# 20171130/Equivariant-NN-Zoo

Measured on AMD Instinct MI355X. Metric: molecules/s forward+backward, QM9 config_energy batch, higher is better.
Workload: dtype f32

## Files before the change

equivariant-nn-zoo_amd/csrc/e3k_graph.hip:

```cpp
#include "e3k_common.h"

namespace e3k {

__global__ __launch_bounds__(256) void csr_count_kernel(const int64_t* __restrict__ edge_index, int64_t E, int32_t N,
                                                        int32_t* __restrict__ src, int32_t* __restrict__ dst,
                                                        int32_t* __restrict__ dst_ptr, int32_t* __restrict__ src_ptr,
                                                        int32_t* __restrict__ bad) {
  const int64_t e = (int64_t)blockIdx.x * 256 + threadIdx.x;
  if (e >= E) return;
  int64_t s = edge_index[e], d = edge_index[E + e];
  if (s < 0 || s >= N || d < 0 || d >= N) {
    *bad = 1;
    s = d = 0;
  }
  src[e] = (int32_t)s;
  dst[e] = (int32_t)d;
  atomicAdd(src_ptr + s + 1, 1);
  atomicAdd(dst_ptr + d + 1, 1);
}

__global__ __launch_bounds__(1024) void csr_scan_kernel(int32_t* __restrict__ dst_ptr, int32_t* __restrict__ src_ptr,
                                                        int32_t* __restrict__ dst_cur, int32_t* __restrict__ src_cur, int32_t N) {
  int32_t* ptr = blockIdx.x == 0 ? dst_ptr : src_ptr;
  int32_t* cur = blockIdx.x == 0 ? dst_cur : src_cur;
// ... 129 lines not shown
      bounds[2 * k] = acc;
      bounds[2 * k + 1] = count[k];
      acc += count[k];
    }
  }
  __syncthreads();
  for (int base = 0; base < R; base += 1024) {
    const int i = base + t;
    int k = -1;
    if (i < R) {
      const int64_t kk = key[i];
      k = (kk >= 0 && kk < K) ? (int)kk : -1;
    }
    int rank = 0;
    for (int q = 0; q < K; ++q) {
      const unsigned long long b = __ballot(k == q);
      if (k == q) rank = __popcll(b & ((1ull << lane) - 1ull));
      if (lane == 0) hist[w][q] = __popcll(b);
    }
    __syncthreads();
    int before[GR_EPT];
#pragma unroll
    for (int j = 0; j < GR_EPT; ++j) {
      const int e = t + 1024 * j, tw = e / K, tq = e - tw * K;
      before[j] = 0;
      if (e < 16 * K)
        for (int v = 0; v < tw; ++v) before[j] += hist[v][tq];
    }
    __syncthreads();
    int total_q[GR_EPT];
#pragma unroll
    for (int j = 0; j < GR_EPT; ++j) {
      const int e = t + 1024 * j, tw = e / K, tq = e - tw * K;
      total_q[j] = 0;
      if (e < 16 * K) {
        if (tw == 15) total_q[j] = before[j] + hist[15][tq];
        hist[tw][tq] = before[j];
      }
    }
    __syncthreads();
    if (k >= 0) perm[start[k] + running[k] + hist[w][k] + rank] = i;
    __syncthreads();
#pragma unroll
    for (int j = 0; j < GR_EPT; ++j) {
      const int e = t + 1024 * j, tw = e / K, tq = e - tw * K;
      if (e < 16 * K && tw == 15) running[tq] += total_q[j];
    }
    __syncthreads();
  }
  if (t < K) reps[t] = count[t] > 0 ? perm[start[t]] : 0;
}
}

namespace e3k {
__global__ __launch_bounds__(256) void edge_records_kernel(const int32_t* __restrict__ perm, const int32_t* __restrict__ nbr,
                                                           const int32_t* __restrict__ bin, const float* __restrict__ coef,
                                                           const float* __restrict__ sh, int d_sh, int64_t E, int32_t* __restrict__ rec) {
  const int64_t q = (int64_t)blockIdx.x * 256 + threadIdx.x;
  if (q >= E * 16) return;
  const int64_t t = q >> 4;
  const int f = (int)(q & 15);
  const int e = perm[t];
  int32_t v = 0;
  if (f == 0) v = nbr[e];
  else if (f == 1) v = bin ? bin[e] : 0;
  else if (f < 6) v = coef ? __float_as_int(coef[4 * (int64_t)e + (f - 2)]) : 0;
  else if (f < 15) v = (f - 6) < d_sh ? __float_as_int(sh[(int64_t)e * d_sh + (f - 6)]) : 0;
  else v = e;
  rec[q] = v;
}
}

extern "C" int e3k_edge_records(const int32_t* perm, const int32_t* nbr, const int32_t* bin, const float* coef, const float* sh,
                                int32_t d_sh, int64_t E, int32_t* rec, void* stream) {
  if (E < 0 || d_sh <= 0 || d_sh > 9 || (bin != nullptr) != (coef != nullptr)) return E3K_ERR_INVALID;
  if (E >= 0x7fffffffLL) return E3K_ERR_UNSUPPORTED;
  if (E == 0) return E3K_OK;
  if (!perm || !nbr || !sh || !rec || (reinterpret_cast<uintptr_t>(rec) & 63)) return E3K_ERR_INVALID;
  hipLaunchKernelGGL(e3k::edge_records_kernel, dim3((unsigned)((E * 16 + 255) / 256)), dim3(256), 0, (hipStream_t)stream, perm, nbr, bin,
                     coef, sh, d_sh, E, rec);
  E3K_CHECK_LAUNCH();
  return E3K_OK;
}

extern "C" int e3k_group_rows(const int64_t* key, int64_t R, int32_t K, int32_t* perm, int32_t* bounds, int64_t* reps,
                              int32_t* bad_flag, void* stream) {
  if (R < 0 || K <= 0) return E3K_ERR_INVALID;
  if (K > e3k::GR_MAXK || R >= 0x7fffffffLL) return E3K_ERR_UNSUPPORTED;
  if (!bounds || !reps || !bad_flag || (R > 0 && (!key || !perm))) return E3K_ERR_INVALID;
  hipStream_t st = (hipStream_t)stream;
  hipLaunchKernelGGL(e3k::group_rows_kernel, dim3(1), dim3(1024), 0, st, key, (int32_t)R, K, perm, bounds, reps, bad_flag);
  E3K_CHECK_LAUNCH();
  return E3K_OK;
}
```

equivariant-nn-zoo_amd/csrc/e3k_rtable.hip:

```cpp
#include "e3k_common.h"
#include "e3k_rtable_bwd.h"

namespace e3k {


constexpr int RT_CHUNK = 1024;
__global__ __launch_bounds__(256) void rtable_bins_rank_kernel(const float* __restrict__ r, const int64_t* __restrict__ key, int64_t E,
                                                               float h_inv, int32_t K, int32_t KT, int32_t* __restrict__ bin,
                                                               float* __restrict__ coef, int32_t* __restrict__ lrank,
                                                               int32_t* __restrict__ chunk_hist, int32_t* __restrict__ bad) {
  extern __shared__ int32_t hist_all[];
  const int lane = threadIdx.x & 63, wv = threadIdx.x >> 6;
  int32_t* hist = hist_all + wv * (KT + 1);
  const int64_t chunk = blockIdx.x;
  for (int b = threadIdx.x; b < 4 * (KT + 1); b += 256) hist_all[b] = 0;
  __syncthreads();
  constexpr int PER_WAVE = RT_CHUNK / 4 / 64;
  const int64_t base = chunk * RT_CHUNK + (int64_t)wv * (RT_CHUNK / 4);
  int my_bin[PER_WAVE], my_rank[PER_WAVE];
#pragma unroll
  for (int it = 0; it < PER_WAVE; ++it) {
    const int64_t e = base + it * 64 + lane;
    const bool live = e < E;
    int i = 1;
    if (live) {
      const float raw = r[e] * h_inv;
      float x = raw < 0.f ? 0.f : (raw > (float)K ? (float)K : raw);
      i = (int)x;
      i = i < 1 ? 1 : (i > K - 2 ? K - 2 : i);
      const float t = x - (float)i;
      const float tm1 = t - 1.f, tm2 = t - 2.f, tp1 = t + 1.f;
      float4 c;
      c.x = -t * tm1 * tm2 * (1.f / 6.f);
      c.y = tp1 * tm1 * tm2 * 0.5f;
      c.z = -tp1 * t * tm2 * 0.5f;
      c.w = tp1 * t * tm1 * (1.f / 6.f);
      if (key) {
        const int64_t kk = key[e];
        const int nk = (KT + 1) / (K + 1);
        const bool in_range = kk >= 0 && kk < nk;
        i += in_range ? (int)kk * (K + 1) : 0;
        if (!in_range && bad) atomicOr(bad, 8);
      }
      bin[e] = i;
      *reinterpret_cast<float4*>(coef + 4 * e) = c;
    }
    unsigned long long todo = __ballot(live);
    int rank = 0;
    while (todo) {
      const int leader = __ffsll((long long)todo) - 1;
      const int b = __shfl(i, leader, 64);
      const unsigned long long same = __ballot(live && i == b) & todo;
      const int seen = hist[b];
      if (live && i == b) rank = seen + __popcll(same & ((1ull << lane) - 1ull));
      if (lane == leader) hist[b] = seen + __popcll(same);
      todo &= ~same;
    }
    my_bin[it] = live ? i : -1;
    my_rank[it] = rank;
  }
  __syncthreads();
#pragma unroll
  for (int it = 0; it < PER_WAVE; ++it) {
    if (my_bin[it] < 0) continue;
    int before = 0;
    for (int w = 0; w < wv; ++w) before += hist_all[w * (KT + 1) + my_bin[it]];
    lrank[base + it * 64 + lane] = my_rank[it] + before;
  }
  for (int b = threadIdx.x; b <= KT; b += 256)
    chunk_hist[chunk * (KT + 1) + b] = hist_all[b] + hist_all[(KT + 1) + b] + hist_all[2 * (KT + 1) + b] + hist_all[3 * (KT + 1) + b];
}

__global__ __launch_bounds__(1024) void rtable_bins_scan_kernel(int32_t* __restrict__ chunk_hist, int32_t n_chunks, int32_t K,
                                                                int32_t* __restrict__ ptr, int32_t* __restrict__ seg) {
  __shared__ int32_t wave_tot[2][16];
  __shared__ int32_t carry[2];
  const int t = threadIdx.x, lane = t & 63, w = t >> 6;
  if (t < 2) carry[t] = 0;
  __syncthreads();
  for (int base = 0; base <= K; base += 1024) {
    const int b = base + t;
    int32_t cnt = 0;
    if (b <= K) {
      for (int c = 0; c < n_chunks; ++c) {
        const int32_t v = chunk_hist[(int64_t)c * (K + 1) + b];
        chunk_hist[(int64_t)c * (K + 1) + b] = cnt;
        cnt += v;
      }
    }
    const int32_t sg = (cnt + RT_SEG - 1) / RT_SEG;
    int32_t x = cnt, y = sg;
#pragma unroll
    for (int off = 1; off < 64; off <<= 1) {
      const int32_t xx = __shfl_up(x, off, 64), yy = __shfl_up(y, off, 64);
      if (lane >= off) x += xx, y += yy;
    }
    if (lane == 63) wave_tot[0][w] = x, wave_tot[1][w] = y;
    __syncthreads();
    int32_t bx = carry[0], by = carry[1];
    for (int k = 0; k < w; ++k) bx += wave_tot[0][k], by += wave_tot[1][k];
    if (b <= K) {
      ptr[b] = bx + x - cnt;
      seg[b] = by + y - sg;
      if (b == K) ptr[K + 1] = bx + x, seg[K + 1] = by + y;
    }
    __syncthreads();
    if (t == 1023) carry[0] = bx + x, carry[1] = by + y;
    __syncthreads();
  }
}

__global__ __launch_bounds__(256) void rtable_bins_place_kernel(const int32_t* __restrict__ bin, const int32_t* __restrict__ lrank,
                                                                const int32_t* __restrict__ chunk_off, const int32_t* __restrict__ ptr,
                                                                int64_t E, int32_t K, int32_t* __restrict__ perm) {
  const int64_t e = (int64_t)blockIdx.x * 256 + threadIdx.x;
  if (e >= E) return;
  const int b = bin[e];
  perm[ptr[b] + chunk_off[(e / RT_CHUNK) * (K + 1) + b] + lrank[e]] = (int32_t)e;
}

__global__ __launch_bounds__(256) void rtable_interp_fwd_kernel(const float* __restrict__ T, const int32_t* __restrict__ perm,
                                                                const int32_t* __restrict__ bin, const float* __restrict__ coef,
                                                                int64_t E, int32_t W, float* __restrict__ w,
                                                                const float* __restrict__ T2, float* __restrict__ w2) {
  const int64_t p = (int64_t)blockIdx.x * 4 + (threadIdx.x >> 6);
  if (p >= E) return;
  const int lane = threadIdx.x & 63;
  const int e = uniform(perm[p]);
  const int i = uniform(bin[e]);
  const float* __restrict__ cp = coef + 4 * (int64_t)e;
  const float c0 = __uint_as_float(uniform((int)__float_as_uint(cp[0]))), c1 = __uint_as_float(uniform((int)__float_as_uint(cp[1])));
  const float c2 = __uint_as_float(uniform((int)__float_as_uint(cp[2]))), c3 = __uint_as_float(uniform((int)__float_as_uint(cp[3])));
  const float4* __restrict__ a = reinterpret_cast<const float4*>(T + (int64_t)(i - 1) * W);
  const float4* __restrict__ b = reinterpret_cast<const float4*>(T + (int64_t)i * W);
  const float4* __restrict__ c = reinterpret_cast<const float4*>(T + (int64_t)(i + 1) * W);
  const float4* __restrict__ d = reinterpret_cast<const float4*>(T + (int64_t)(i + 2) * W);
  float4* __restrict__ o = reinterpret_cast<float4*>(w + (int64_t)e * W);
  for (int q = lane; q < (W >> 2); q += 64) {
    const float4 va = a[q], vb = b[q], vc = c[q], vd = d[q];
    float4 v;
// ... 254 lines not shown
}

extern "C" int e3k_rtable_pack(const float* T, int32_t K, int32_t W, void* P, void* stream) {
  if (K < 4 || W <= 0) return E3K_ERR_INVALID;
  if (!T || !P) return E3K_ERR_INVALID;
  const int64_t q = (int64_t)(K + 1) * W;
  hipLaunchKernelGGL(e3k::rtable_pack_kernel, dim3((unsigned)((q + 255) / 256)), dim3(256), 0, (hipStream_t)stream, T, K, W,
                     static_cast<uint32_t*>(P));
  E3K_CHECK_LAUNCH();
  return E3K_OK;
}

extern "C" int e3k_rtable_pack_multi(const float* const* T, int32_t K, const int32_t* W, void* const* P, int32_t n, void* stream) {
  if (K < 4 || n < 0 || n > 16) return E3K_ERR_INVALID;
  if (n == 0) return E3K_OK;
  if (!T || !W || !P) return E3K_ERR_INVALID;
  e3k::PackMulti a{};
  int32_t wmax = 0;
  for (int i = 0; i < n; ++i) {
    if (!T[i] || !P[i] || W[i] <= 0) return E3K_ERR_INVALID;
    a.T[i] = T[i];
    a.P[i] = static_cast<uint32_t*>(P[i]);
    a.W[i] = W[i];
    wmax = W[i] > wmax ? W[i] : wmax;
  }
  const int64_t q = (int64_t)(K + 1) * wmax;
  hipLaunchKernelGGL(e3k::rtable_pack_multi_kernel, dim3((unsigned)((q + 255) / 256), (unsigned)n), dim3(256), 0, (hipStream_t)stream, a, K);
  E3K_CHECK_LAUNCH();
  return E3K_OK;
}

extern "C" int e3k_rtable_interp_packed(const void* P, const int32_t* bin_perm, const int32_t* bin, const float* coef, int64_t E,
                                        int32_t K, int32_t W, float* w, void* stream) {
  if (E < 0 || K < 4 || W <= 0) return E3K_ERR_INVALID;
  if (E >= 0x7fffffffLL) return E3K_ERR_UNSUPPORTED;
  if (E == 0) return E3K_OK;
  if (!P || !bin_perm || !bin || !coef || !w) return E3K_ERR_INVALID;
  hipLaunchKernelGGL(e3k::rtable_interp_packed_kernel, dim3((unsigned)((E + 3) / 4)), dim3(256), 0, (hipStream_t)stream,
                     static_cast<const uint32_t*>(P), bin_perm, bin, coef, E, W, w);
  E3K_CHECK_LAUNCH();
  return E3K_OK;
}

extern "C" int64_t e3k_rtable_bins_workspace_ints(int64_t E, int32_t K) {
  const int64_t n_chunks = (E + e3k::RT_CHUNK - 1) / e3k::RT_CHUNK;
  return E + n_chunks * ((int64_t)K + 1);
}

static int rtable_bins_impl(const float* r, const int64_t* key, int32_t n_keys, int64_t E, float h_inv, int32_t K, int32_t* bin,
                            float* coef, int32_t* bin_ptr, int32_t* bin_seg, int32_t* bin_perm, int32_t* workspace, int32_t* bad_flag,
                            void* stream) {
  if (E < 0 || K < 4 || !(h_inv > 0.f) || n_keys < 1) return E3K_ERR_INVALID;
  const int64_t KT64 = (int64_t)n_keys * (K + 1) - 1;
  if (KT64 > 4000 || E >= 0x7fffffffLL) return E3K_ERR_UNSUPPORTED;
  const int32_t KT = (int32_t)KT64;
  if (!bin_ptr || !bin_seg) return E3K_ERR_INVALID;
  if (E > 0 && (!r || !bin || !coef || !bin_perm || !workspace)) return E3K_ERR_INVALID;
  hipStream_t st = (hipStream_t)stream;
  const int64_t n_chunks = (E + e3k::RT_CHUNK - 1) / e3k::RT_CHUNK;
  int32_t* lrank = workspace;
  int32_t* chunk_hist = workspace + E;
  if (E > 0)
    hipLaunchKernelGGL(e3k::rtable_bins_rank_kernel, dim3((unsigned)n_chunks), dim3(256), sizeof(int32_t) * 4 * (KT + 1), st, r, key, E,
                       h_inv, K, KT, bin, coef, lrank, chunk_hist, bad_flag);
  hipLaunchKernelGGL(e3k::rtable_bins_scan_kernel, dim3(1), dim3(1024), 0, st, chunk_hist, (int32_t)n_chunks, KT, bin_ptr, bin_seg);
  if (E > 0)
    hipLaunchKernelGGL(e3k::rtable_bins_place_kernel, dim3((unsigned)((E + 255) / 256)), dim3(256), 0, st, bin, lrank, chunk_hist,
                       bin_ptr, E, KT, bin_perm);
  E3K_CHECK_LAUNCH();
  return E3K_OK;
}

extern "C" int e3k_rtable_bins(const float* r, int64_t E, float h_inv, int32_t K, int32_t* bin, float* coef,
                               int32_t* bin_ptr, int32_t* bin_seg, int32_t* bin_perm, int32_t* workspace, void* stream) {
  return rtable_bins_impl(r, nullptr, 1, E, h_inv, K, bin, coef, bin_ptr, bin_seg, bin_perm, workspace, nullptr, stream);
}

extern "C" int e3k_rtable_bins_keyed(const float* r, const int64_t* key, int32_t n_keys, int64_t E, float h_inv, int32_t K,
                                     int32_t* bin, float* coef, int32_t* bin_ptr, int32_t* bin_seg, int32_t* bin_perm,
                                     int32_t* workspace, int32_t* bad_flag, void* stream) {
  if (E > 0 && !key) return E3K_ERR_INVALID;
  return rtable_bins_impl(r, key, n_keys, E, h_inv, K, bin, coef, bin_ptr, bin_seg, bin_perm, workspace, bad_flag, stream);
}

extern "C" int e3k_rtable_interp_fwd(const float* T, const int32_t* bin_perm, const int32_t* bin, const float* coef, int64_t E,
                                     int32_t K, int32_t W, float* w, void* stream) {
  if (E < 0 || K < 4 || W <= 0) return E3K_ERR_INVALID;
  if (W % 4 || E >= 0x7fffffffLL) return E3K_ERR_UNSUPPORTED;
  if (E == 0) return E3K_OK;
  if (!T || !bin_perm || !bin || !coef || !w) return E3K_ERR_INVALID;
  hipLaunchKernelGGL(e3k::rtable_interp_fwd_kernel, dim3((unsigned)((E + 3) / 4)), dim3(256), 0, (hipStream_t)stream, T, bin_perm,
                     bin, coef, E, W, w, (const float*)nullptr, (float*)nullptr);
  E3K_CHECK_LAUNCH();
  return E3K_OK;
}

extern "C" int e3k_rtable_interp_fwd2(const float* T, const float* T2, const int32_t* bin_perm, const int32_t* bin, const float* coef,
                                      int64_t E, int32_t K, int32_t W, float* w, float* w2, void* stream) {
  if (E < 0 || K < 4 || W <= 0) return E3K_ERR_INVALID;
  if (W % 4 || E >= 0x7fffffffLL) return E3K_ERR_UNSUPPORTED;
  if (E == 0) return E3K_OK;
  if (!T || !T2 || !bin_perm || !bin || !coef || !w || !w2) return E3K_ERR_INVALID;
  hipLaunchKernelGGL(e3k::rtable_interp_fwd_kernel, dim3((unsigned)((E + 3) / 4)), dim3(256), 0, (hipStream_t)stream, T, bin_perm,
                     bin, coef, E, W, w, T2, w2);
  E3K_CHECK_LAUNCH();
  return E3K_OK;
}
// ... 27 lines not shown
```

equivariant-nn-zoo_amd/e3_layers_amd/backend/radial_table.py:

```python
from __future__ import annotations

import os
import weakref
from typing import Optional

import torch

from .tuning import knob as _knob

from . import lib as L
from . import memo, ops

ENABLED = _knob("E3K_RADIAL_TABLE")
KNOTS = _knob("E3K_RADIAL_KNOTS")
KNOTS_SLOPE = _knob("E3K_RADIAL_KNOTS_SLOPE")
MIN_EDGES_PER_KNOT = _knob("E3K_RADIAL_MIN_EDGES_PER_KNOT")
KNOTS_MAX = _knob("E3K_RADIAL_KNOTS_MAX")
_KNOTS_AT_START = (int(KNOTS), int(KNOTS_SLOPE))
REFINEMENTS = 0
KEYED = _knob("E3K_RADIAL_TABLE_KEYED")


def layout(r_max: float, target: int):
    import math

    m = math.ceil(math.log2(max(int(target), 4) / float(r_max)) - 1e-9)
    h = 2.0 ** (-m)
    return max(int(math.ceil(float(r_max) / h - 1e-9)), 4), h


class KnotBins:

    __slots__ = ("bin", "coef", "ptr", "perm", "seg", "knots", "spacing", "blocks", "_buf", "_rec", "__weakref__")

    def __init__(self, bin, coef, ptr, perm, seg, knots: int, spacing: float, buf=None):
        self.bin, self.coef, self.ptr, self.perm, self.seg, self.knots, self.spacing = bin, coef, ptr, perm, seg, int(knots), float(spacing)
        self._buf = buf
        self._rec = {}
        self.blocks = 1

    def records(self, topo, sh: torch.Tensor, walk: str) -> torch.Tensor:
        perm, nbr = (topo.dst_perm, topo.src) if walk == "dst" else (topo.src_perm, topo.dst)
        key = (walk, sh.data_ptr(), sh._version, perm.data_ptr())
        hit = self._rec.get(key)
        if hit is None:
            sh = L.f32c(sh.detach())
            e = perm.numel()
            if sh.dim() != 2 or sh.shape[0] != e or sh.shape[1] > 9:
                raise ValueError(f"edge records take [E, <= 9] spherical harmonics, got {tuple(sh.shape)} for {e} edges")
            rec = torch.empty(max(e, 1), 16, dtype=torch.int32, device=sh.device)
            L.check(L.load().e3k_edge_records(L.ptr(perm), L.ptr(nbr), L.ptr(self.bin), L.ptr(self.coef), L.ptr(sh), sh.shape[1], e,
                                              L.ptr(rec), L.stream_ptr()), "e3k_edge_records")
            hit = self._rec[key] = (rec, sh)
        return hit[0]

    def tensors(self):
        return (self._buf, self.coef) if self._buf is not None else (self.bin, self.coef, self.ptr, self.perm, self.seg)

    def __iter__(self):
        return iter(self.tensors())


def build_bins(r: torch.Tensor, r_max: float, target: int, key: Optional[torch.Tensor] = None, n_keys: int = 1) -> KnotBins:
    knots, h = layout(r_max, target)
    r = L.f32c(r.detach().reshape(-1))
    L.require_cuda(r)
    e, dev = r.numel(), r.device
    lib = L.load()
    n_keys = int(n_keys) if key is not None else 1
    last = n_keys * (knots + 1) - 1
    sizes = [e, e, last + 2, last + 2, int(lib.e3k_rtable_bins_workspace_ints(e, last))]
    buf = torch.empty(sum(sizes), dtype=torch.int32, device=dev)
    bin32, perm, ptr, seg, work = torch.split(buf, sizes)
    coef = torch.empty(e, 4, dtype=torch.float32, device=dev)
    if key is None:
        L.check(lib.e3k_rtable_bins(L.ptr(r), e, 1.0 / h, knots, L.ptr(bin32), L.ptr(coef), L.ptr(ptr), L.ptr(seg), L.ptr(perm),
                                    L.ptr(work), L.stream_ptr()), "e3k_rtable_bins")
    else:
        key = key.detach().reshape(-1)
        if key.dtype != torch.int64 or not key.is_contiguous():
            key = key.long().contiguous()
        if key.numel() != e:
            raise ValueError(f"{key.numel()} keys for {e} radii")
        from . import graph as _graph

        capturing = torch.cuda.is_current_stream_capturing()
        flag = _graph._capture_flags.get(dev.index) if capturing else _graph.persistent_flag(dev)
        L.check(lib.e3k_rtable_bins_keyed(L.ptr(r), L.ptr(key), n_keys, e, 1.0 / h, knots, L.ptr(bin32), L.ptr(coef), L.ptr(ptr),
                                          L.ptr(seg), L.ptr(perm), L.ptr(work), L.ptr(flag), L.stream_ptr()), "e3k_rtable_bins_keyed")
        if flag is not None:
            _graph.report_persistent(dev)
    bins = KnotBins(bin32, coef, ptr, perm, seg, last, h, buf)
    bins.blocks = n_keys
    return bins


class RadialSource:

    __slots__ = ("module", "r", "version", "knots", "knots_slope", "_bins", "_knot_basis", "_stack", "__weakref__")

    def __init__(self, module, r: torch.Tensor, version: int = 0, prepared: Optional[dict] = None):
        self.module, self.r, self.version = weakref.ref(module), r, int(version)
        self.knots, self.knots_slope = int(KNOTS), int(KNOTS_SLOPE)
        self._bins = dict(prepared) if prepared else {}
        self._knot_basis = {}
        self._stack = {}

# ... 408 lines not shown
```

equivariant-nn-zoo_amd/e3_layers_amd/nn/message_passing.py:

```python
from __future__ import annotations

import math
import os
import weakref

from typing import Callable, Dict, Optional, Tuple

import torch

from ..backend.tuning import knob as _knob
from torch import Tensor

from ..backend import conv_block, conv_native, memo, ops, radial_table
from ..backend.graph import get_topology
from ..o3 import Irrep, Irreps
from ..utils.utils import _is_mapping, activations, build, tp_path_exists
from .core import (FullyConnectedNet, FullyConnectedTensorProduct, Gate, Linear, NormActivation, get_row_key, irreps_blocks,
                   row_groups)
from .pointwise import LayerNormalization, TensorProductExpansion
from .sequential import Module


FWD_FORK = _knob("E3K_FWD_FORK")
FORK_MIN_EDGES = _knob("E3K_FORK_MIN_EDGES")
# ... 377 lines not shown
        if nmp is not None and fork and nmp.conv._fork_pays(n_edges, table is not None):
            plan_n = nmp._block_plan()
            if plan_n is not None and (nmp.conv.sc is None) == (conv.sc is None):
                fc_n = list(nmp.conv.fc.children())
                same_path = (table is not None) == radial_table.applicable(data["edge_radial"], fc_n[-1].weight)
                if fc_n[0].weight.shape[0] == radial.shape[1] and same_path:
                    nxt = (plan_n, fc_n[-1].weight, [m.weight for m in fc_n[:-1]])
        y = conv_block.conv_block(x, attrs, radial, sh, plan, topo, groups, bool(getattr(x, "_e3k_cf", False)), out_cf, fork,
                                  conv.linear_1.weight, conv.tp.linear.weight, conv.sc.weight if conv.sc is not None else None,
                                  fc[-1].weight, [m.weight for m in fc[:-1]], table=table, nxt=nxt, m_pre=m_pre)
        return y

    def _forward_block_addend(self, data, x, sh, radial, out_cf: bool):
        plan = self._block_plan(addend=True) if BLOCK_ADDEND else None
        if plan is None:
            return None
        conv = self.conv
        x_cf = x if getattr(x, "_e3k_cf", False) else ops.relayout(x, conv._in_blocks, True)
        sc_out = conv.sc(x_cf, data["node_attrs"])
        topo = get_topology(data, x.shape[0])
        fc = list(conv.fc.children())
        table = None
        if radial_table.applicable(radial, fc[-1].weight):
            src = radial_table.source_of(radial)
            table = src.bins()
            radial = src.knot_basis()
        fork = bool(FWD_FORK and conv._fork_pays(data["edge_radial"].shape[0], table is not None)
                    and not torch.cuda.is_current_stream_capturing())
        if fork:
            main = ops.current_stream(x.device)
            side = ops.side_stream(x.device)
            with ops.on_stream(side, main):
                radial = _stream_alias(radial, side)
        return conv_block.conv_block(x_cf, None, radial, sh, plan, topo, None, True, out_cf, fork,
                                     conv.linear_1.weight, conv.tp.linear.weight, None,
                                     fc[-1].weight, [m.weight for m in fc[:-1]], table=table, m_pre=sc_out)

    def prepare_batch(self, network, data, avail) -> None:
        from ..backend.graph import GraphTopo

        if not conv_native.TP_TABLE:
            return
        inv = {loc: g for g, loc in self.input_key_mapping.items()}
        sh_key, rad_key = inv.get("edge_spherical"), inv.get("edge_radial")
        sh = data.get(sh_key) if sh_key in avail else None
        topo = GraphTopo.from_dict(data)
        if sh is None or topo is None or not sh.is_cuda or sh.dim() != 2 or sh.shape[1] > 9 or sh.shape[0] != topo.num_edges:
            return
        for _, layer in network.layers:
            if rad_key in getattr(layer, "output_key_mapping", {}).values() and hasattr(layer, "basis"):
                r_key = next((g for g, loc in layer.input_key_mapping.items() if loc == "input"), None)
                bins = radial_table.prepared_bins(data[r_key], layer.basis.r_max) if (r_key in avail and r_key in data) else None
                for b in (bins or {}).values():
                    b.records(topo, sh, "dst")
                    if torch.is_grad_enabled() or self.training:
                        b.records(topo, sh, "src")

    def forward(self, data: Dict[str, Tensor], attrs: Dict[str, Tuple[str, str]]):
        old_x = data["input_features"]
        blk = self._forward_block(data, bool(self._emit_cf))
        if blk is not None:
            if self._emit_cf:
                if self.normalize:
                    blk = self.norm({"input": blk}, attrs)[0]["output"]
                blk._e3k_cf = True
                return ({"output_features": blk},
                        {"output_features": (attrs["input_features"][0], self.irreps_out["output_features"])})
            output = blk
            if self.resnet:
                output = old_x + output
            if self.normalize:
                output = self.norm({"input": output}, attrs)[0]["output"]
            return ({"output_features": output},
                    {"output_features": (attrs["input_features"][0], self.irreps_out["output_features"])})
        if isinstance(self.conv, FactorizedConvolution) and self.conv.reduce:
            conv_cf = self.conv.forward_cf(data)
        else:
            if getattr(old_x, "_e3k_cf", False):
                raise RuntimeError("cf hand-over reached a convolution that cannot take it (container bug)")
            out, _ = self.conv(data, attrs)
            conv_cf = ops.relayout(out["output_features"], tuple(irreps_blocks(self.equivariant_nonlin.irreps_in)), True)
        if self._emit_cf:
            output = self.equivariant_nonlin(conv_cf, out_cf=True)
            if self.normalize:
                output = self.norm({"input": output}, attrs)[0]["output"]
            output._e3k_cf = True
            return ({"output_features": output},
                    {"output_features": (attrs["input_features"][0], self.irreps_out["output_features"])})
        output = self.equivariant_nonlin(conv_cf)
        if self.resnet:
            output = old_x + output
        if self.normalize:
            output = self.norm({"input": output}, attrs)[0]["output"]
        return ({"output_features": output},
                {"output_features": (attrs["input_features"][0], self.irreps_out["output_features"])})
```

equivariant-nn-zoo_amd/e3_layers_amd/run/graph_step.py:

```python
from __future__ import annotations

import os
from typing import Any, Callable

import numpy as np
import torch

from ..backend import memo


class CapturedStep:
    def __init__(self, fn: Callable[[], Any], warmup: int = 3, device=None, generators=()):
        if not torch.cuda.is_available():
            raise RuntimeError("CapturedStep needs a HIP device: there is no CPU fallback for graph replay")
        self.fn = fn
        self.generators = tuple(generators)
        self.dev = torch.device("cuda", torch.cuda.current_device()) if device is None else torch.device(device)
        self.recaptures = 0
        self._capture(max(1, warmup))

    def _eager(self, n: int):
        dev = self.dev
        side = torch.cuda.Stream(dev)
        side.wait_stream(torch.cuda.current_stream(dev))
# ... 85 lines not shown
        elif name == "_n_nodes":
            tensors[name] = torch.full_like(v, n_nodes)
        elif name == "_n_edges":
            tensors[name] = torch.full_like(v, n_edges)
        elif torch.is_tensor(v) and (like.attrs.get(name, ("",))[0] == "node"
                                     or (name not in like.attrs and v.dim() >= 1 and v.shape[0] == like[key].shape[0])):
            tensors[name] = v[:1].expand(n_nodes, *v.shape[1:]).clone()
        elif name == "edge_cell_shift":
            tensors[name] = v.new_zeros((n_edges,) + tuple(v.shape[1:]))
        elif torch.is_tensor(v) and like.attrs.get(name, ("",))[0] == "edge":
            tensors[name] = (v[:1].expand(n_edges, *v.shape[1:]).clone() if v.shape[0] else v.new_zeros((n_edges,) + tuple(v.shape[1:])))
        elif torch.is_tensor(v):
            tensors[name] = torch.zeros_like(v)
        else:
            tensors[name] = v
    return Data(attrs=dict(like.attrs), **tensors)


def pad_batch(batch, n_cap: int, e_cap: int, key: str = "pos"):
    from ..data.data import Batch
    from ..data.loader import samples_of

    dev = batch[key].device
    samples = samples_of(batch)
    n, e = int(batch[key].shape[0]), int(batch["edge_index"].shape[1])
    if n_cap < n + 2 or e_cap < e:
        raise ValueError(f"batch with {n} nodes / {e} edges does not fit the bucket ({n_cap}, {e_cap}; two ghost nodes are the minimum)")
    samples.append(ghost_sample(samples[0], n_cap - n, e_cap - e, key))
    out = Batch.from_data_list(samples, attrs=dict(samples[0].attrs))
    w = torch.full((len(samples), 1), 1.0 / (len(samples) - 1), dtype=torch.float32)
    w[-1] = 0.0
    out["_graph_weight"] = w
    out.attrs["_graph_weight"] = ("graph", "1x0e")
    wn = torch.zeros(n_cap, 1, dtype=torch.float32)
    wn[:n] = 1.0 / n
    out["_node_weight"] = wn
    out.attrs["_node_weight"] = ("node", "1x0e")
    return out.to(dev)


GHOST_DEGREE = 16


def ghost_node_capacity(n: int, ghost_edges: int, multiple: int = 32) -> int:
    return -(-(n + max(2, -(-ghost_edges // GHOST_DEGREE))) // multiple) * multiple


def bucket_capacity(sizes, node_multiple: int = 32, edge_multiple: int = 1024):
    e_cap = -(-max(e for _, e in sizes) // edge_multiple) * edge_multiple
    return max(ghost_node_capacity(n, e_cap - e, node_multiple) for n, e in sizes), e_cap


def copy_into(static, padded, keys, hint: str = "") -> None:
    by_dtype = {}
    for k in keys:
        dst, src = static[k], padded[k]
        if dst.shape != src.shape:
            raise ValueError(f"{k}: {tuple(src.shape)} does not fit the captured {tuple(dst.shape)} (another bucket?"
                             f"{' ' + hint if hint else ''})")
        if src.device == dst.device and src.dtype == dst.dtype and src.is_contiguous() and dst.is_contiguous():
            pair = by_dtype.setdefault(dst.dtype, ([], []))
            pair[0].append(dst)
            pair[1].append(src)
        else:
            dst.copy_(src, non_blocking=True)
    for dsts, srcs in by_dtype.values():
        torch._foreach_copy_(dsts, srcs)


class BucketedStep:

    def __init__(self, fn: Callable[[Any], Any], example, warmup: int = 3, generators=(), tail: Callable[[], Any] = None):
        self.tail = tail
        self.static = example.clone()
        self.keys = [k for k in self.static.keys() if torch.is_tensor(self.static[k])]

        def captured_fn():
            memo.forget(self.static)
            return fn(self.static.view())

        self.captured = CapturedStep(captured_fn, warmup=warmup, generators=generators)

    @property
    def recaptures(self) -> int:
        return self.captured.recaptures

    def __call__(self, padded):
        copy_into(self.static, padded, self.keys)
        out = self.captured()
        if self.tail is not None:
            self.tail()
        return out


def stream_beside(main, candidates: int = 6):
    dev = main.device
    busy = torch.empty(16 << 20, device=dev)
    tiny = torch.zeros(64, device=dev)
    pool = [torch.cuda.Stream(dev) for _ in range(candidates)]
    for st in pool:
        torch.cuda.synchronize(dev)
        with torch.cuda.stream(main):
            for _ in range(40):
                busy.mul_(1.0)
            main_done = torch.cuda.Event()
            main_done.record(main)
        with torch.cuda.stream(st):
            tiny.add_(1.0)
            mine = torch.cuda.Event()
            mine.record(st)
        mine.synchronize()
        beside = not main_done.query()
        torch.cuda.synchronize(dev)
        if beside:
            return st
    return pool[0]


class PipelinedBucketedStep:

# ... 206 lines not shown
```

include/e3k.h:

```cpp
#ifndef E3K_H
#define E3K_H

#include <stdint.h>

#ifdef __cplusplus
extern "C" {
#endif

#define E3K_OK 0
#define E3K_ERR_INVALID (-1)
#define E3K_ERR_LAUNCH (-2)
#define E3K_ERR_UNSUPPORTED (-3)

#define E3K_TP_MAXQ 8
#define E3K_NARROW_MAX_SLOTS 48

const char* e3k_strerror(int code);
int e3k_version(void);
void e3k_tp_limits(int* l1max, int* l2max, int* l3max);

typedef struct {
  const float* A;
  const float* A2;
  const float* B;
// ... 116 lines not shown
                       const float* g_out, const int32_t* dst, const int32_t* src_ptr, const int32_t* src_perm, int64_t N,
                       int64_t E, float* g_x, void* stream);
int e3k_tp_fwd_ptable(const e3k_tp_plan* plan, const float* x, const void* P, const int32_t* erec_dst, const int32_t* dst_ptr,
                      int64_t N, int64_t E, float* out, void* stream);
int e3k_tp_bwd_x_ptable(const e3k_tp_plan* plan, const void* P, const int32_t* erec_src, const float* g_out, const int32_t* src_ptr,
                        int64_t N, int64_t E, float* g_x, void* stream);
int e3k_tp_bwd_xw_ptable(const e3k_tp_plan* plan, const float* x, const void* P, const int32_t* erec_src, const float* g_out,
                         const int32_t* src_ptr, int64_t N, int64_t E, float* g_x, float* g_w, void* stream);
int e3k_tp_scalar_supported(const e3k_tp_plan* plan);
int e3k_tp_bwd_xw_scalar_ptable(const e3k_tp_plan* plan, const float* x, const void* P, int32_t table_w, const int32_t* table_off,
                                const int32_t* erec_src, const float* g_out, const int32_t* src_ptr, int64_t N, int64_t E, float* g_x,
                                float* g_w, void* stream);
int e3k_tp_masked_supported(const e3k_tp_plan* plan);
int e3k_tp_bwd_xw_masked_ptable(const e3k_tp_plan* plan, const float* x, const void* P, int32_t table_w, const int32_t* live_col,
                                const int32_t* erec_src, const float* g_out, const int32_t* src_ptr, int64_t N, int64_t E, float* g_x,
                                float* g_w, void* stream);
int e3k_expand_columns(const float* src, int64_t rows, int32_t w_src, int32_t w_dst, const int32_t* src_col, const int32_t* dst_col,
                       const int32_t* len, int32_t n_ranges, float* dst, void* stream);
int e3k_tp_bwd_xw(const e3k_tp_plan* plan, const float* x, const float* sh, const float* w, const float* g_out, const int32_t* dst,
                  const int32_t* src_ptr, const int32_t* src_perm, int64_t N, int64_t E, float* g_x, float* g_w, void* stream);
int e3k_tp_table2_supported(const e3k_tp_plan* plan);
int e3k_tp_second_order_streamed_supported(const e3k_tp_plan* plan);
int e3k_tp_bwd_e_table(const e3k_tp_plan* plan, const float* x, const float* sh, const float* T, const float* D,
                       const int32_t* bin, const float* coef, const float* g_out, const int32_t* src, const int32_t* dst_ptr,
                       const int32_t* dst_perm, int64_t N, int64_t E, float* g_sh, float* g_r, float* g_w, float* e_partials,
                       void* stream);
int64_t e3k_tp_edge_partials_floats(const e3k_tp_plan* plan, int64_t E);
int e3k_tp_fwd_jvp_table(const e3k_tp_plan* plan, const float* x, const float* x2, const float* sh, const float* sh2,
                         const float* T, const float* D, const int32_t* bin, const float* coef, const float* s2,
                         const int32_t* src, const int32_t* dst_ptr, const int32_t* dst_perm, int64_t N, int64_t E, float* out,
                         void* stream);
int e3k_tp_bwd_x_dual_table(const e3k_tp_plan* plan, const float* sh, const float* sh2, const float* T, const float* D,
                            const int32_t* bin, const float* coef, const float* s2, const float* g_out, const int32_t* dst,
                            const int32_t* src_ptr, const int32_t* src_perm, int64_t N, int64_t E, float* g_x, void* stream);
int e3k_tp_bwd_xe(const e3k_tp_plan* plan, const float* x, const float* sh, const float* w, const float* dw, const float* g_out,
                  const int32_t* dst, const int32_t* src_ptr, const int32_t* src_perm, int64_t N, int64_t E, float* g_x, float* g_sh,
                  float* g_r, float* g_w, float* e_partials, void* stream);
int e3k_tp_bwd_xw_dual(const e3k_tp_plan* plan, const float* x, const float* x2, const float* sh, const float* sh2, const float* w,
                       const float* dw, const float* s2, const float* g_out, const int32_t* dst, const int32_t* src_ptr,
                       const int32_t* src_perm, int64_t N, int64_t E, float* g_x, float* g_w, float* g_w_plain, void* stream);
int e3k_tp_bwd_w_dual(const e3k_tp_plan* plan, const float* x, const float* x2, const float* sh, const float* sh2,
                      const float* g_out, const int32_t* src, const int32_t* dst_ptr, const int32_t* dst_perm, int64_t N, int64_t E,
                      float* g_w, void* stream);
int e3k_tp_bwd_x(const e3k_tp_plan* plan, const float* sh, const float* w, const float* g_out, const int32_t* dst,
                 const int32_t* src_ptr, const int32_t* src_perm, int64_t N, int64_t E, float* g_x, void* stream);

int64_t e3k_csr_workspace_ints(int64_t N, int64_t E);
int e3k_csr_build(const int64_t* edge_index, int64_t N, int64_t E, int32_t* src, int32_t* dst, int32_t* dst_ptr,
                  int32_t* dst_perm, int32_t* src_ptr, int32_t* src_perm, int32_t* workspace, int32_t* bad_flag,
                  void* stream);

int e3k_edge_records(const int32_t* perm, const int32_t* nbr, const int32_t* bin, const float* coef, const float* sh, int32_t d_sh,
                     int64_t E, int32_t* rec, void* stream);

int e3k_group_rows(const int64_t* key, int64_t R, int32_t K, int32_t* perm, int32_t* bounds, int64_t* reps,
                   int32_t* bad_flag, void* stream);

#define E3K_COLLATE_NODE 0
#define E3K_COLLATE_EDGE 1
#define E3K_COLLATE_GRAPH 2
#define E3K_COLLATE_EDGE_INDEX 3
#define E3K_COLLATE_NODE_SEGMENT 4
#define E3K_COLLATE_EDGE_SEGMENT 5
#define E3K_COLLATE_NODE_WEIGHT 6
#define E3K_COLLATE_GHOST_FIRST 0
#define E3K_COLLATE_GHOST_TABLE 1
#define E3K_COLLATE_MAX_FIELDS 16
typedef struct {
  int32_t kind;
  int32_t ghost;
  int64_t row_bytes;
  const void* src;
  void* dst;
  const void* table;
  int64_t src_ld;
  int64_t dst_ld;
} e3k_collate_field;
int64_t e3k_collate_work_ints(int32_t G);
int e3k_collate_plan(const int32_t* ids, int32_t G, const int64_t* node_off, const int64_t* edge_off, int64_t S, int64_t n_cap,
                     int64_t e_cap, int64_t* work, int64_t* n_nodes, int64_t* n_edges, float* graph_weight, int32_t* flag,
                     void* stream);
int e3k_collate_gather(const e3k_collate_field* fields, int32_t n_fields, int32_t G, int64_t n_cap, int64_t e_cap,
                       const int64_t* work, void* stream);

int64_t e3k_rtable_bins_workspace_ints(int64_t E, int32_t K);
int e3k_rtable_bins(const float* r, int64_t E, float h_inv, int32_t K, int32_t* bin, float* coef,
                    int32_t* bin_ptr, int32_t* bin_seg, int32_t* bin_perm, int32_t* workspace, void* stream);
int e3k_rtable_bins_keyed(const float* r, const int64_t* key, int32_t n_keys, int64_t E, float h_inv, int32_t K, int32_t* bin,
                          float* coef, int32_t* bin_ptr, int32_t* bin_seg, int32_t* bin_perm, int32_t* workspace, int32_t* bad_flag,
                          void* stream);
int e3k_rtable_interp_fwd(const float* T, const int32_t* bin_perm, const int32_t* bin, const float* coef, int64_t E, int32_t K,
                          int32_t W, float* w, void* stream);
int e3k_rtable_interp_fwd2(const float* T, const float* T2, const int32_t* bin_perm, const int32_t* bin, const float* coef, int64_t E,
                           int32_t K, int32_t W, float* w, float* w2, void* stream);
int64_t e3k_rtable_bwd_workspace_floats(int64_t E, int32_t K, int32_t W);
int e3k_rtable_interp_bwd(const float* g_w, const float* coef, const float* scale, const int32_t* bin_ptr,
                          const int32_t* bin_seg, const int32_t* bin_perm, int64_t E, int32_t K, int32_t W, float* workspace,
                          float* g_T, int32_t accumulate, void* stream);
int e3k_wgrad_with_table_bwd(const e3k_gemm_segment* segments, int32_t n_segments, const float* g_w, const float* coef,
                             const float* scale, const int32_t* bin_ptr, const int32_t* bin_seg, const int32_t* bin_perm, int64_t E,
                             int32_t K, int32_t W, float* workspace, float* g_T, int32_t accumulate, void* stream);

int e3k_rtable_pack(const float* T, int32_t K, int32_t W, void* P, void* stream);
int e3k_rtable_pack_multi(const float* const* T, int32_t K, const int32_t* W, void* const* P, int32_t n, void* stream);
int e3k_rtable_interp_packed(const void* P, const int32_t* bin_perm, const int32_t* bin, const float* coef, int64_t E, int32_t K,
                             int32_t W, float* w, void* stream);

int e3k_rtable_guard(const float* const* tables, float* const* states, float* const* scratch, const int32_t* widths, int32_t n,
                     int32_t rows, float floor_rel, float col_weight, int32_t packed, void* stream);

int e3k_act_fwd(const float* x, int64_t n, int32_t act, float cst, float* y, void* stream);
int e3k_act_bwd(const float* x, const float* g_y, int64_t n, int32_t act, float cst, float* g_x, void* stream);
int e3k_act_bwd_from_output(const float* y, const float* g_y, int64_t n, int32_t act, float cst, float* g_x,
                            void* stream);
int e3k_act_bwd2(const float* x, const float* g_y, const float* g_hat, int64_t n, int32_t act, float cst,
                 float* g_gy, float* g_x, void* stream);

typedef struct {
  int32_t off, mul, dim, _pad;
} e3k_block;
int e3k_relayout(const float* x, int64_t rows, int32_t row_dim, const e3k_block* blocks, int32_t n_blocks,
                 int32_t to_cf, float* y, void* stream);

typedef struct {
  int32_t kind;
  int32_t in_off;
  int32_t gate_off;
  int32_t out_off;
  int32_t mul, dim;
  int32_t act;
  float cst;
} e3k_gate_seg;
int e3k_gate_fwd(const float* x, int64_t rows, int32_t in_dim, int32_t out_dim, const e3k_gate_seg* segs,
                 int32_t n_segs, int32_t out_cf, float* y, void* stream);
int e3k_gate_bwd(const float* x, const float* g_y, const float* g_y2, int64_t rows, int32_t in_dim, int32_t out_dim,
                 const e3k_gate_seg* segs, int32_t n_segs, int32_t out_cf, float* g_x, void* stream);
// ... 329 lines not shown
```

Baseline: 95530.

## Batch per-step copies and edge-record builds; speed up bin ranking and scan

```diff
diff --git a/equivariant-nn-zoo_amd/csrc/e3k_graph.hip b/equivariant-nn-zoo_amd/csrc/e3k_graph.hip
--- a/equivariant-nn-zoo_amd/csrc/e3k_graph.hip
+++ b/equivariant-nn-zoo_amd/csrc/e3k_graph.hip
@@ -205,22 +205,14 @@
 }
 }
 
+#include "e3k_records.h"
 namespace e3k {
 __global__ __launch_bounds__(256) void edge_records_kernel(const int32_t* __restrict__ perm, const int32_t* __restrict__ nbr,
                                                            const int32_t* __restrict__ bin, const float* __restrict__ coef,
                                                            const float* __restrict__ sh, int d_sh, int64_t E, int32_t* __restrict__ rec) {
   const int64_t q = (int64_t)blockIdx.x * 256 + threadIdx.x;
   if (q >= E * 16) return;
-  const int64_t t = q >> 4;
-  const int f = (int)(q & 15);
-  const int e = perm[t];
-  int32_t v = 0;
-  if (f == 0) v = nbr[e];
-  else if (f == 1) v = bin ? bin[e] : 0;
-  else if (f < 6) v = coef ? __float_as_int(coef[4 * (int64_t)e + (f - 2)]) : 0;
-  else if (f < 15) v = (f - 6) < d_sh ? __float_as_int(sh[(int64_t)e * d_sh + (f - 6)]) : 0;
-  else v = e;
-  rec[q] = v;
+  rec[q] = record_word(perm, nbr, bin, coef, sh, d_sh, q >> 4, (int)(q & 15));
 }
 }
 
diff --git a/equivariant-nn-zoo_amd/csrc/e3k_prepare.hip b/equivariant-nn-zoo_amd/csrc/e3k_prepare.hip
--- /dev/null
+++ b/equivariant-nn-zoo_amd/csrc/e3k_prepare.hip
@@ -0,0 +1,83 @@
+#include "e3k_common.h"
+#include "e3k_records.h"
+
+namespace e3k {
+struct CopyArgs {
+  e3k_copy_field f[E3K_MULTI_COPY_MAX_FIELDS];
+};
+
+template <typename T>
+__device__ __forceinline__ void copy_units(char* __restrict__ dst, const char* __restrict__ src, int64_t bytes, int64_t tid,
+                                           int64_t n_threads) {
+  const int64_t n = bytes / (int64_t)sizeof(T);
+  const T* __restrict__ s = reinterpret_cast<const T*>(src);
+  T* __restrict__ d = reinterpret_cast<T*>(dst);
+  for (int64_t i = tid; i < n; i += n_threads) d[i] = s[i];
+  const int64_t done = n * (int64_t)sizeof(T);
+  if (tid < bytes - done) dst[done + tid] = src[done + tid];
+}
+
+__global__ __launch_bounds__(256) void multi_copy_kernel(const CopyArgs a) {
+  const e3k_copy_field& f = a.f[blockIdx.y];
+  const int64_t bytes = f.bytes;
+  const int64_t tid = (int64_t)blockIdx.x * 256 + threadIdx.x, n_threads = (int64_t)gridDim.x * 256;
+  char* dst = static_cast<char*>(f.dst);
+  const char* src = static_cast<const char*>(f.src);
+  const uintptr_t both = reinterpret_cast<uintptr_t>(dst) | reinterpret_cast<uintptr_t>(src);
+  if ((both & 15) == 0) copy_units<uint4>(dst, src, bytes, tid, n_threads);
+  else if ((both & 3) == 0) copy_units<uint32_t>(dst, src, bytes, tid, n_threads);
+  else copy_units<uint8_t>(dst, src, bytes, tid, n_threads);
+}
+}
+
+extern "C" int e3k_multi_copy(const e3k_copy_field* fields, int32_t n_fields, void* stream) {
+  if (n_fields < 0 || (n_fields > 0 && !fields)) return E3K_ERR_INVALID;
+  for (int i = 0; i < n_fields; ++i)
+    if (fields[i].bytes < 0 || (fields[i].bytes > 0 && (!fields[i].src || !fields[i].dst))) return E3K_ERR_INVALID;
+  e3k::CopyArgs a = {};
+  int n = 0;
+  int64_t longest = 0;
+  for (int i = 0; i <= n_fields; ++i) {
+    if (i < n_fields && fields[i].bytes > 0) {
+      a.f[n++] = fields[i];
+      longest = fields[i].bytes > longest ? fields[i].bytes : longest;
+    }
+    if (n == E3K_MULTI_COPY_MAX_FIELDS || (i == n_fields && n > 0)) {
+      int64_t blocks = (longest + 16 * 256 - 1) / (16 * 256);
+      blocks = blocks > 512 ? 512 : blocks;
+      hipLaunchKernelGGL(e3k::multi_copy_kernel, dim3((unsigned)blocks, (unsigned)n), dim3(256), 0, (hipStream_t)stream, a);
+      E3K_CHECK_LAUNCH();
+      n = 0;
+      longest = 0;
+    }
+  }
+  return E3K_OK;
+}
+
+namespace e3k {
+__global__ __launch_bounds__(256) void edge_records_both_kernel(const int32_t* __restrict__ dst_perm, const int32_t* __restrict__ src,
+                                                                const int32_t* __restrict__ src_perm, const int32_t* __restrict__ dst,
+                                                                const int32_t* __restrict__ bin, const float* __restrict__ coef,
+                                                                const float* __restrict__ sh, int d_sh, int64_t E,
+                                                                int32_t* __restrict__ rec_dst, int32_t* __restrict__ rec_src) {
+  const int64_t q = (int64_t)blockIdx.x * 256 + threadIdx.x;
+  if (q >= E * 16) return;
+  const bool by_src = blockIdx.y != 0;
+  (by_src ? rec_src : rec_dst)[q] = record_word(by_src ? src_perm : dst_perm, by_src ? dst : src, bin, coef, sh, d_sh, q >> 4, (int)(q & 15));
+}
+}
+
+extern "C" int e3k_edge_records_both(const int32_t* dst_perm, const int32_t* src, const int32_t* src_perm, const int32_t* dst,
+                                     const int32_t* bin, const float* coef, const float* sh, int32_t d_sh, int64_t E,
+                                     int32_t* rec_dst, int32_t* rec_src, void* stream) {
+  if (E < 0 || d_sh <= 0 || d_sh > 9 || (bin != nullptr) != (coef != nullptr)) return E3K_ERR_INVALID;
+  if (E >= 0x7fffffffLL) return E3K_ERR_UNSUPPORTED;
+  if (E == 0) return E3K_OK;
+  if (!dst_perm || !src || !src_perm || !dst || !sh || !rec_dst || !rec_src || rec_dst == rec_src ||
+      ((reinterpret_cast<uintptr_t>(rec_dst) | reinterpret_cast<uintptr_t>(rec_src)) & 63))
+    return E3K_ERR_INVALID;
+  hipLaunchKernelGGL(e3k::edge_records_both_kernel, dim3((unsigned)((E * 16 + 255) / 256), 2), dim3(256), 0, (hipStream_t)stream,
+                     dst_perm, src, src_perm, dst, bin, coef, sh, d_sh, E, rec_dst, rec_src);
+  E3K_CHECK_LAUNCH();
+  return E3K_OK;
+}
diff --git a/equivariant-nn-zoo_amd/csrc/e3k_records.h b/equivariant-nn-zoo_amd/csrc/e3k_records.h
--- /dev/null
+++ b/equivariant-nn-zoo_amd/csrc/e3k_records.h
@@ -0,0 +1,15 @@
+#pragma once
+#include "e3k_common.h"
+
+namespace e3k {
+__device__ __forceinline__ int32_t record_word(const int32_t* __restrict__ perm, const int32_t* __restrict__ nbr,
+                                               const int32_t* __restrict__ bin, const float* __restrict__ coef,
+                                               const float* __restrict__ sh, int d_sh, int64_t t, int f) {
+  const int e = perm[t];
+  if (f == 0) return nbr[e];
+  if (f == 1) return bin ? bin[e] : 0;
+  if (f < 6) return coef ? __float_as_int(coef[4 * (int64_t)e + (f - 2)]) : 0;
+  if (f < 15) return (f - 6) < d_sh ? __float_as_int(sh[(int64_t)e * d_sh + (f - 6)]) : 0;
+  return e;
+}
+}
diff --git a/equivariant-nn-zoo_amd/csrc/e3k_rtable.hip b/equivariant-nn-zoo_amd/csrc/e3k_rtable.hip
--- a/equivariant-nn-zoo_amd/csrc/e3k_rtable.hip
+++ b/equivariant-nn-zoo_amd/csrc/e3k_rtable.hip
@@ -5,6 +5,21 @@
 
 
 constexpr int RT_CHUNK = 1024;
+constexpr int RT_MAX_ROW = 4000;
+constexpr int RT_KNOT_BITS = 12;
+
+__device__ __forceinline__ unsigned long long lanes_of_same_knot(int knot) {
+  static_assert(RT_MAX_ROW < (1 << RT_KNOT_BITS), "a live knot must fit RT_KNOT_BITS bits");
+  unsigned long long same = ~0ull;
+#pragma unroll
+  for (int bit = 0; bit <= RT_KNOT_BITS; ++bit) {
+    const bool mine = (knot >> bit) & 1;
+    const unsigned long long set = __ballot(mine);
+    same &= mine ? set : ~set;
+  }
+  return same;
+}
+
 __global__ __launch_bounds__(256) void rtable_bins_rank_kernel(const float* __restrict__ r, const int64_t* __restrict__ key, int64_t E,
                                                                float h_inv, int32_t K, int32_t KT, int32_t* __restrict__ bin,
                                                                float* __restrict__ coef, int32_t* __restrict__ lrank,
@@ -45,18 +60,18 @@
       bin[e] = i;
       *reinterpret_cast<float4*>(coef + 4 * e) = c;
     }
-    unsigned long long todo = __ballot(live);
+    const int knot = live ? i : -1;
+    const unsigned long long same = lanes_of_same_knot(knot);
+    const int below = __popcll(same & ((1ull << lane) - 1ull));
+    const bool later = (same >> lane) != 1ull;
     int rank = 0;
-    while (todo) {
-      const int leader = __ffsll((long long)todo) - 1;
-      const int b = __shfl(i, leader, 64);
-      const unsigned long long same = __ballot(live && i == b) & todo;
-      const int seen = hist[b];
-      if (live && i == b) rank = seen + __popcll(same & ((1ull << lane) - 1ull));
-      if (lane == leader) hist[b] = seen + __popcll(same);
-      todo &= ~same;
-    }
-    my_bin[it] = live ? i : -1;
+    if (live) {
+      rank = hist[knot] + below;
+      if (!later) hist[knot] = rank + 1;
+    }
+    __builtin_amdgcn_fence(__ATOMIC_ACQ_REL, "wavefront");
+    __builtin_amdgcn_wave_barrier();
+    my_bin[it] = knot;
     my_rank[it] = rank;
   }
   __syncthreads();
@@ -82,10 +97,18 @@
     const int b = base + t;
     int32_t cnt = 0;
     if (b <= K) {
-      for (int c = 0; c < n_chunks; ++c) {
-        const int32_t v = chunk_hist[(int64_t)c * (K + 1) + b];
-        chunk_hist[(int64_t)c * (K + 1) + b] = cnt;
-        cnt += v;
+      constexpr int SCAN_BATCH = 8;
+      int32_t* __restrict__ col = chunk_hist + b;
+      const int64_t ld = K + 1;
+      for (int c0 = 0; c0 < n_chunks; c0 += SCAN_BATCH) {
+        int32_t v[SCAN_BATCH];
+#pragma unroll
+        for (int u = 0; u < SCAN_BATCH; ++u) v[u] = c0 + u < n_chunks ? col[(c0 + u) * ld] : 0;
+#pragma unroll
+        for (int u = 0; u < SCAN_BATCH; ++u) {
+          if (c0 + u < n_chunks) col[(c0 + u) * ld] = cnt;
+          cnt += v[u];
+        }
       }
     }
     const int32_t sg = (cnt + RT_SEG - 1) / RT_SEG;
@@ -446,7 +469,7 @@
                             void* stream) {
   if (E < 0 || K < 4 || !(h_inv > 0.f) || n_keys < 1) return E3K_ERR_INVALID;
   const int64_t KT64 = (int64_t)n_keys * (K + 1) - 1;
-  if (KT64 > 4000 || E >= 0x7fffffffLL) return E3K_ERR_UNSUPPORTED;
+  if (KT64 > e3k::RT_MAX_ROW || E >= 0x7fffffffLL) return E3K_ERR_UNSUPPORTED;
   const int32_t KT = (int32_t)KT64;
   if (!bin_ptr || !bin_seg) return E3K_ERR_INVALID;
   if (E > 0 && (!r || !bin || !coef || !bin_perm || !workspace)) return E3K_ERR_INVALID;
diff --git a/equivariant-nn-zoo_amd/e3_layers_amd/backend/radial_table.py b/equivariant-nn-zoo_amd/e3_layers_amd/backend/radial_table.py
--- a/equivariant-nn-zoo_amd/e3_layers_amd/backend/radial_table.py
+++ b/equivariant-nn-zoo_amd/e3_layers_amd/backend/radial_table.py
@@ -53,6 +53,21 @@
                                               L.ptr(rec), L.stream_ptr()), "e3k_edge_records")
             hit = self._rec[key] = (rec, sh)
         return hit[0]
+
+    def records_both(self, topo, sh: torch.Tensor) -> None:
+        keys = [(walk, sh.data_ptr(), sh._version, perm.data_ptr()) for walk, perm in (("dst", topo.dst_perm), ("src", topo.src_perm))]
+        e = topo.dst_perm.numel()
+        if any(k in self._rec for k in keys) or e == 0 or sh.dim() != 2 or sh.shape[0] != e or sh.shape[1] > 9:
+            self.records(topo, sh, "dst")
+            self.records(topo, sh, "src")
+            return
+        sh = L.f32c(sh.detach())
+        rec = torch.empty(2, e, 16, dtype=torch.int32, device=sh.device)
+        L.check(L.load().e3k_edge_records_both(L.ptr(topo.dst_perm), L.ptr(topo.src), L.ptr(topo.src_perm), L.ptr(topo.dst),
+                                               L.ptr(self.bin), L.ptr(self.coef), L.ptr(sh), sh.shape[1], e, L.ptr(rec[0]),
+                                               L.ptr(rec[1]), L.stream_ptr()), "e3k_edge_records_both")
+        for k, r in zip(keys, rec):
+            self._rec[k] = (r, sh)
 
     def tensors(self):
         return (self._buf, self.coef) if self._buf is not None else (self.bin, self.coef, self.ptr, self.perm, self.seg)
diff --git a/equivariant-nn-zoo_amd/e3_layers_amd/nn/message_passing.py b/equivariant-nn-zoo_amd/e3_layers_amd/nn/message_passing.py
--- a/equivariant-nn-zoo_amd/e3_layers_amd/nn/message_passing.py
+++ b/equivariant-nn-zoo_amd/e3_layers_amd/nn/message_passing.py
@@ -453,9 +453,10 @@
                 r_key = next((g for g, loc in layer.input_key_mapping.items() if loc == "input"), None)
                 bins = radial_table.prepared_bins(data[r_key], layer.basis.r_max) if (r_key in avail and r_key in data) else None
                 for b in (bins or {}).values():
-                    b.records(topo, sh, "dst")
                     if torch.is_grad_enabled() or self.training:
-                        b.records(topo, sh, "src")
+                        b.records_both(topo, sh)
+                    else:
+                        b.records(topo, sh, "dst")
 
     def forward(self, data: Dict[str, Tensor], attrs: Dict[str, Tuple[str, str]]):
         old_x = data["input_features"]
diff --git a/equivariant-nn-zoo_amd/e3_layers_amd/run/graph_step.py b/equivariant-nn-zoo_amd/e3_layers_amd/run/graph_step.py
--- a/equivariant-nn-zoo_amd/e3_layers_amd/run/graph_step.py
+++ b/equivariant-nn-zoo_amd/e3_layers_amd/run/graph_step.py
@@ -161,20 +161,28 @@
 
 
 def copy_into(static, padded, keys, hint: str = "") -> None:
-    by_dtype = {}
+    by_dtype, native = {}, {}
     for k in keys:
         dst, src = static[k], padded[k]
         if dst.shape != src.shape:
             raise ValueError(f"{k}: {tuple(src.shape)} does not fit the captured {tuple(dst.shape)} (another bucket?"
                              f"{' ' + hint if hint else ''})")
         if src.device == dst.device and src.dtype == dst.dtype and src.is_contiguous() and dst.is_contiguous():
-            pair = by_dtype.setdefault(dst.dtype, ([], []))
+            pair = native.setdefault(dst.device, ([], [])) if dst.is_cuda else by_dtype.setdefault(dst.dtype, ([], []))
             pair[0].append(dst)
             pair[1].append(src)
         else:
             dst.copy_(src, non_blocking=True)
     for dsts, srcs in by_dtype.values():
         torch._foreach_copy_(dsts, srcs)
+    for dev, (dsts, srcs) in native.items():
+        from ..backend import lib as L
+
+        table = (L.CopyField * len(dsts))(*[L.CopyField(s.data_ptr(), d.data_ptr(), d.numel() * d.element_size())
+                                           for d, s in zip(dsts, srcs)])
+        with torch.cuda.device(dev):
+            L.check(L.load().e3k_multi_copy(table, len(dsts), L.stream_ptr()), "e3k_multi_copy")
+        torch.autograd.graph.increment_version(dsts)
 
 
 class BucketedStep:
diff --git a/include/e3k.h b/include/e3k.h
--- a/include/e3k.h
+++ b/include/e3k.h
@@ -192,6 +192,9 @@
 
 int e3k_edge_records(const int32_t* perm, const int32_t* nbr, const int32_t* bin, const float* coef, const float* sh, int32_t d_sh,
                      int64_t E, int32_t* rec, void* stream);
+int e3k_edge_records_both(const int32_t* dst_perm, const int32_t* src, const int32_t* src_perm, const int32_t* dst,
+                          const int32_t* bin, const float* coef, const float* sh, int32_t d_sh, int64_t E, int32_t* rec_dst,
+                          int32_t* rec_src, void* stream);
 
 int e3k_group_rows(const int64_t* key, int64_t R, int32_t K, int32_t* perm, int32_t* bounds, int64_t* reps,
                    int32_t* bad_flag, void* stream);
@@ -222,6 +225,14 @@
                      void* stream);
 int e3k_collate_gather(const e3k_collate_field* fields, int32_t n_fields, int32_t G, int64_t n_cap, int64_t e_cap,
                        const int64_t* work, void* stream);
+
+#define E3K_MULTI_COPY_MAX_FIELDS 32
+typedef struct {
+  const void* src;
+  void* dst;
+  int64_t bytes;
+} e3k_copy_field;
+int e3k_multi_copy(const e3k_copy_field* fields, int32_t n_fields, void* stream);
 
 int64_t e3k_rtable_bins_workspace_ints(int64_t E, int32_t K);
 int e3k_rtable_bins(const float* r, int64_t E, float h_inv, int32_t K, int32_t* bin, float* coef,
```

New measurement: 95810, median of 6. About the same (+0.3%).
